# RohanVKashyap/resolution-pde

Measured on AMD Instinct MI355X. Metric: training samples/sec, FFNO2D NS 256^2, higher is better.
Workload: dtype f32; 1 GPU; FFNO2D(1,1,width=64,n_layers=4,n_modes=20,factor=4,ff_weight_norm,n_ff_layers=3,layer_norm,dropout=0.1) train step on [B,1,256,256] Gaussian random fields (BASELINE configs[2]); batch_per_gpu=32, global_batch=32, optimizer=AdamW lr=1e-3 (rpde.optim.FlatAdamW: torch.optim.AdamW's rule, one kernel), parallelism=single, grad_bucket_bytes=6828576, target=input advanced by a fixed spectral filter (utils/synthetic.py:advance)

## Files before the change

resolution-pde_amd/csrc/feedforward.hip:

```cpp
#include "rpde_internal.h"
#include "pointwise.h"
#include "gemm_kernel.h"
#include "ff_fused.h"
#include "ff_bwd_split.h"
#include "wgrad_h2.h"
#include "thin_linear.h"
#include "conv_small.h"

#include <vector>

namespace rpde {


static inline int ff_in(const rpde_ff_params* p, int l) { return l == 0 ? p->dim : p->dim * p->factor; }
static inline int ff_out(const rpde_ff_params* p, int l) { return l == p->n_layers - 1 ? p->dim : p->dim * p->factor; }

static inline int wgrad_split(long P, int out_f, int in_f) {
  const int tiles = ((out_f + 127) / 128) * ((in_f + 127) / 128);
  long s = 768 / tiles;
  const long cap = (P + 127) / 128;
  if (s > cap) s = cap;
  if (s < 1) s = 1;
  if (s > 1024) s = 1024;
  return (int)s;
// ... 86 lines not shown
  const size_t b = wgrad_h2_slab_floats(P, out_f, in_f);
  if (b > a) a = b;
  if (in_f <= 4 && thin_linear_ok(in_f, out_f) && thin_outer_ws_floats(P, in_f, out_f) > a) a = thin_outer_ws_floats(P, in_f, out_f);
  if (out_f <= 4 && thin_linear_ok(out_f, in_f) && thin_outer_ws_floats(P, out_f, in_f) > a) a = thin_outer_ws_floats(P, out_f, in_f);
  return a;
}

static rpde_ff_params ff_dims(int dim, int factor, int n_layers) {
  rpde_ff_params q;
  memset(&q, 0, sizeof(q));
  q.dim = dim; q.factor = factor; q.n_layers = n_layers;
  return q;
}
static int ff_hid(const rpde_ff_params& q) { return q.n_layers > 1 ? q.dim * q.factor : q.dim; }

struct FfBwdWork {
  float *buf0, *buf1, *small, *tailws, *dz3 = nullptr, *part = nullptr;
  void* fimg = nullptr;
  std::vector<float*> slabs, csum, wt;
  FfBwdWork(Arena& ar, const rpde_ff_params& q, long P, bool fused) {
    const int L = q.n_layers > 0 ? q.n_layers : 0, hid = ff_hid(q);
    slabs.resize(L); csum.resize(L); wt.resize(L);
    buf0 = ar.take((size_t)P * hid);
    buf1 = ar.take((size_t)P * hid);
    for (int l = 0; l < L; ++l) slabs[l] = ar.take(wgrad_ws_floats(P, ff_in(&q, l), ff_out(&q, l)));
    for (int l = 0; l < L; ++l) csum[l] = ar.take((size_t)(colsum_tiles(P) + REDUCE_CHUNKS) * hid);
    for (int l = 0; l < L; ++l) wt[l] = ar.take(ff_wimg_floats(hid));
    small = ar.take(colsum_ws_floats(P, hid));
    tailws = ar.take(ff_tail_bwd_ws_floats(P, q.dim));
    if (!fused) return;
    dz3 = ar.take((size_t)P * q.dim);
    part = ar.take(ff3_fused_bwd_part_floats());
    fimg = ar.take(ff3_fused_ws_floats());
  }
};
struct FfFwdImgs {
  std::vector<float*> wimg;
  FfFwdImgs(Arena& ar, const rpde_ff_params& q, int n) : wimg(n > 0 ? n : 0) { for (float*& w : wimg) w = ar.take(ff_wimg_floats(ff_hid(q))); }
};
struct FfFusedImg {
  void* img;
  explicit FfFusedImg(Arena& ar) : img(ar.take(ff3_fused_ws_floats())) {}
};

}

using namespace rpde;

extern "C" {

size_t rpde_feedforward_ws_bytes(int64_t P, int dim, int factor, int n_layers) {
  const rpde_ff_params q = ff_dims(dim, factor, n_layers);
  const size_t general = ws_measure<FfBwdWork>(q, (long)P, false);
  return ff3_fused_ok(&q, (long)P) ? ws_max(general, ws_measure<FfBwdWork>(q, (long)P, true)) : general;
}

size_t rpde_feedforward_fwd_ws_bytes(int dim, int factor, int n_layers) {
  return ws_max(ws_measure<FfFwdImgs>(ff_dims(dim, factor, n_layers), n_layers), ws_measure<FfFusedImg>());
}

int rpde_feedforward_is_fused(int dim, int factor, int n_layers, int64_t P) {
  const rpde_ff_params q = ff_dims(dim, factor, n_layers);
  return ff3_fused_ok(&q, (long)P) ? 1 : 0;
}

int rpde_feedforward_prepare(const rpde_ff_params* p, void* prep, size_t prep_bytes, void* stream) {
  RPDE_CHECK_ARG(p && prep, "feedforward_prepare: bad arguments");
  Arena ar(prep, prep_bytes);
  const FfFusedImg f(ar);
  RPDE_CHECK_ARG(ff3_fused_ok(p, 32) && ar.ok(), "feedforward_prepare: shape not fused or buffer too small");
  RPDE_CHECK_ARG(p->weights && p->weights[0] && p->weights[1] && p->weights[2], "feedforward_prepare: null weights");
  return ff3_fused_prepare(p, f.img, as_stream(stream));
}

int rpde_feedforward_fwd_prepared(const rpde_ff_params* p, const float* x, const float* residual, float* out, int64_t P,
                                  const void* prep, size_t prep_bytes, void* stream) {
  RPDE_CHECK_ARG(p && x && out && prep && P > 0 && P < (1L << 31), "feedforward_fwd_prepared: bad arguments");
  Arena ar(const_cast<void*>(prep), prep_bytes);
  const FfFusedImg f(ar);
  RPDE_CHECK_ARG(ff3_fused_ok(p, P) && ar.ok(), "feedforward_fwd_prepared: shape not fused");
  RPDE_CHECK_ARG(!p->layer_norm || (p->ln_gamma && p->ln_beta), "feedforward_fwd_prepared: layer_norm needs gamma/beta");
  RPDE_CHECK_ARG(p->dropout_p == 0.f, "feedforward_fwd_prepared: evaluation only");
  return ff3_fused_fwd(p, x, residual, nullptr, nullptr, out , out, P,
                       f.img, as_stream(stream), true);
}

int rpde_feedforward_fwd(const rpde_ff_params* p, const float* x, const float* residual, float* const* hs,
                         float* const* ds, float* z_last, float* out, int64_t P, void* ws, size_t ws_bytes, void* stream) {
  RPDE_CHECK_ARG(p && x && z_last && out && P > 0, "feedforward_fwd: bad arguments");
  RPDE_CHECK_ARG(p->n_layers >= 1 && p->dim > 0 && p->factor > 0, "feedforward_fwd: bad shape");
  RPDE_CHECK_ARG(P < (1L << 31), "feedforward_fwd: too many points for one call");
  RPDE_CHECK_ARG(p->dropout_p >= 0.f && p->dropout_p < 1.f, "feedforward_fwd: dropout %f", p->dropout_p);
  hipStream_t st = as_stream(stream);
  Arena far(ws, ws_bytes);
  const FfFusedImg fused(far);
  if (ff3_fused_ok(p, P) && far.ok()) {
    RPDE_CHECK_ARG(p->weights[0] && p->weights[1] && p->weights[2], "feedforward_fwd: null weights");
    RPDE_CHECK_ARG(!p->layer_norm || (p->ln_gamma && p->ln_beta), "feedforward_fwd: layer_norm needs gamma/beta");
    return ff3_fused_fwd(p, x, residual, hs, ds, z_last, out, P, fused.img, st);
  }
  RPDE_CHECK_ARG(p->n_layers == 1 || hs, "feedforward_fwd: hidden buffers missing");
  const int L = p->n_layers;
  Arena ar(ws, ws_bytes);
  bool all_imgs = ws != nullptr && L <= SplitJobs::MAX;
  const FfFwdImgs imgs(ar, *p, all_imgs ? L : 1);
  all_imgs = all_imgs && ar.ok();
  float* const* wimg = imgs.wimg.data();
  if (all_imgs) {
    SplitJobs sj;
    for (int l = 0; l < L; ++l) {
      RPDE_CHECK_ARG(p->weights[l], "feedforward_fwd: null layer %d weight", l);
      if (worth_presplit(P, ff_out(p, l), ff_in(p, l))) sj.add(p->weights[l], 1, ff_in(p, l), ff_out(p, l), ff_in(p, l), wimg[l]);
    }
    RPDE_TRY(split_weights_multi(sj, st));
  }
  for (int l = 0; l < L; ++l) {
    const bool last = l == L - 1;
    RPDE_CHECK_ARG(p->weights[l] && (last || hs[l]), "feedforward_fwd: null layer %d buffers", l);
    const float* in = l == 0 ? x : hs[l - 1];
    RPDE_TRY(linear_fwd_impl(in, p->weights[l], p->biases ? p->biases[l] : nullptr, last ? z_last : hs[l], P, ff_in(p, l),
                             ff_out(p, l), last ? RPDE_ACT_IDENTITY : RPDE_ACT_GELU, (last || !ds) ? nullptr : ds[l],
                             p->dropout_p, layer_seed(p->seed, l), st, all_imgs ? wimg[l] : wimg[0], p->seed_epoch, all_imgs));
  }
  return ff_tail_fwd(z_last, residual, out, P, p->dim, p->layer_norm, p->ln_eps, p->ln_gamma, p->ln_beta,
                     make_drop(p->dropout_p, layer_seed(p->seed, L - 1), p->seed_epoch), p->post_act, st);
}

int rpde_feedforward_bwd(const rpde_ff_params* p, const float* x, const float* const* hs, const float* const* ds,
                         const float* z_last, const float* grad_out, float* grad_x, float* const* grad_weights,
                         float* const* grad_biases, float* grad_gamma, float* grad_beta, int64_t P, void* ws,
                         size_t ws_bytes, void* stream) {
  RPDE_CHECK_ARG(p && x && z_last && grad_out && P > 0, "feedforward_bwd: bad arguments");
  RPDE_CHECK_ARG(P < (1L << 31), "feedforward_bwd: too many points for one call");
  const int L = p->n_layers;
  const int hid = ff_hid(*p);
  const bool fused = ff3_fused_ok(p, P) && hs && hs[0] && hs[1];
  RPDE_CHECK_ARG(p->n_layers == 1 || (hs && (ds || fused)), "feedforward_bwd: saved hidden tensors missing");
  RPDE_CARVE("feedforward_bwd", FfBwdWork, wk, ws, ws_bytes, *p, P, fused);
  hipStream_t st = as_stream(stream);
  float *buf0 = wk.buf0, *buf1 = wk.buf1, *small = wk.small, *tailws = wk.tailws;
  const std::vector<float*>&slabs_l = wk.slabs, &csum_l = wk.csum, &wt_l = wk.wt;
  void* wt = wt_l[0];

  if (fused) {
    const int recompute = !(ds && ds[0] && ds[1]);
    const int act_h = recompute ? RPDE_ACT_GELU : RPDE_ACT_IDENTITY;
    float *dz3 = wk.dz3, *part = wk.part;
    void* fimg = wk.fimg;
    int grid = 0;
    const bool both = grad_x && grad_weights && wgrad_h2_dgrad_ok(P, hid, p->dim);
    const bool split = both && !recompute && ff_bwd_split_ok(P, hid, p->dim);
    if (split) {
      FoldJobs folds;
      RPDE_TRY(ff_bwd_split_launch(p, ds, z_last, grad_out, x, dz3, buf0, buf1, grad_x, slabs_l[0], grad_weights[0], part,
                                   &grid, P, fimg, st, &folds));
      RPDE_TRY(linear_wgrad_impl(hs[1], dz3, grad_weights[2], nullptr, P, hid, p->dim, slabs_l[2], small, st, act_h, &folds));
      RPDE_TRY(linear_wgrad_impl(hs[0], buf0, grad_weights[1], nullptr, P, hid, hid, slabs_l[1], small, st, act_h, &folds));
      RPDE_TRY(fold_jobs(folds, st));
    } else {
      RPDE_TRY(ff3_fused_bwd_launch(p, recompute ? hs : ds, recompute, z_last, grad_out, dz3, buf0, buf1, nullptr, part, &grid, P,
                                    fimg, st));
    }
    if (grad_x && !both) RPDE_TRY(linear_dgrad_impl(buf1, p->weights[0], grad_x, P, p->dim, hid, nullptr, nullptr, st, wt));
    if (grad_weights && !split) {
      FoldJobs folds;
      RPDE_TRY(linear_wgrad_impl(hs[1], dz3, grad_weights[2], nullptr, P, hid, p->dim, slabs_l[2], small, st, act_h, &folds));
      RPDE_TRY(linear_wgrad_impl(hs[0], buf0, grad_weights[1], nullptr, P, hid, hid, slabs_l[1], small, st, act_h, &folds));
      if (both) RPDE_TRY(wgrad_h2_dgrad(buf1, x, p->weights[0], grad_weights[0], grad_x, P, p->dim, hid, slabs_l[0], st, &folds));
      else RPDE_TRY(linear_wgrad_impl(x, buf1, grad_weights[0], nullptr, P, p->dim, hid, slabs_l[0], small, st, RPDE_ACT_IDENTITY, &folds));
      RPDE_TRY(fold_jobs(folds, st));
    }
    {
      ReduceSegs sg;
      memset(&sg, 0, sizeof(sg));
      sg.n = FF3_PART; sg.nseg = 5;
      const int off[5] = {0, 256, 512, 576, 640}, len[5] = {hid, hid, p->dim, p->dim, p->dim};
      float* dst[5] = {grad_biases ? grad_biases[0] : nullptr, grad_biases ? grad_biases[1] : nullptr,
                       grad_biases ? grad_biases[2] : nullptr, p->layer_norm ? grad_gamma : nullptr,
                       p->layer_norm ? grad_beta : nullptr};
      for (int k = 0; k < 5; ++k) { sg.off[k] = off[k]; sg.len[k] = len[k]; sg.dst[k] = dst[k]; }
      RPDE_TRY(reduce_slabs_seg(part, grid, FF3_PART, sg, st));
    }
    return RPDE_OK;
  }

  FoldJobs folds;
  float* dz = buf0;
  float* other = buf1;
  int bias_done = 0;
  RPDE_TRY(ff_tail_bwd(z_last, grad_out, dz, P, p->dim, p->layer_norm, p->ln_eps, p->ln_gamma, p->ln_beta,
                       make_drop(p->dropout_p, layer_seed(p->seed, L - 1), p->seed_epoch), p->post_act, grad_gamma, grad_beta,
                       grad_biases ? grad_biases[L - 1] : nullptr, &bias_done, tailws, st, &folds));
  const bool all_imgs = L <= SplitJobs::MAX;
  if (all_imgs) {
    SplitJobs sj;
    for (int l = grad_x ? 0 : 1; l < L; ++l)
      if (worth_presplit(P, ff_in(p, l), ff_out(p, l))) sj.add(p->weights[l], 0, ff_in(p, l), ff_in(p, l), ff_out(p, l), wt_l[l]);
    RPDE_TRY(split_weights_multi(sj, st));
  }
  for (int l = L - 1; l >= 0; --l) {
    const int in_f = ff_in(p, l), out_f = ff_out(p, l);
    const float* in = l == 0 ? x : hs[l - 1];
    float* gb = (grad_biases && !bias_done) ? grad_biases[l] : nullptr;
    RPDE_TRY(linear_wgrad_impl(in, dz, grad_weights ? grad_weights[l] : nullptr, gb, P, in_f, out_f, slabs_l[l], small, st,
                               RPDE_ACT_IDENTITY, &folds));
    bias_done = 0;
    void* img = all_imgs ? wt_l[l] : wt;
    if (l > 0) {
      RPDE_CHECK_ARG(ds[l - 1], "feedforward_bwd: derivative of layer %d was not saved", l - 1);
      const bool fuse = grad_biases && can_fuse_colsum(dz, p->weights[l], other, ds[l - 1], P, in_f, out_f);
      RPDE_TRY(linear_dgrad_impl(dz, p->weights[l], other, P, in_f, out_f, ds[l - 1], fuse ? csum_l[l] : nullptr, st, img, all_imgs));
      if (fuse) {
        const int S = (int)colsum_tiles(P);
        if (!(S <= 4 * REDUCE_CHUNKS && folds.add(csum_l[l], grad_biases[l - 1], in_f, S, in_f)))
          RPDE_TRY(reduce_slabs_2pass(csum_l[l], grad_biases[l - 1], in_f, S, in_f, csum_l[l] + colsum_tiles(P) * in_f, st));
        bias_done = 1;
      }
      float* t = dz; dz = other; other = t;
    } else if (grad_x) {
      RPDE_TRY(linear_dgrad_impl(dz, p->weights[0], grad_x, P, in_f, out_f, nullptr, nullptr, st, img, all_imgs));
    }
  }
  return fold_jobs(folds, st);
}

struct LinearBwdWork {
  float *slabs, *small;
  LinearBwdWork(Arena& ar, long P, int in_f, int out_f)
      : slabs(ar.take(wgrad_ws_floats(P, in_f, out_f))), small(ar.take(colsum_ws_floats(P, out_f))) {}
};

size_t rpde_linear_ws_bytes(int64_t P, int in_f, int out_f) { return ws_measure<LinearBwdWork>((long)P, in_f, out_f); }

int rpde_linear_fwd(const float* x, const float* w, const float* b, float* out, int64_t P, int in_f, int out_f, void* stream) {
  RPDE_CHECK_ARG(x && w && out && P > 0 && in_f > 0 && out_f > 0 && P < (1L << 31), "linear_fwd: bad arguments");
  return linear_fwd_impl(x, w, b, out, P, in_f, out_f, RPDE_ACT_IDENTITY, nullptr, 0.f, 0, as_stream(stream));
}

int rpde_linear_bwd(const float* x, const float* w, const float* grad_out, float* grad_x, float* grad_w, float* grad_b,
                    int64_t P, int in_f, int out_f, void* ws, size_t ws_bytes, void* stream) {
  RPDE_CHECK_ARG(x && w && grad_out && P > 0 && in_f > 0 && out_f > 0 && P < (1L << 31), "linear_bwd: bad arguments");
  RPDE_CARVE("linear_bwd", LinearBwdWork, wk, ws, ws_bytes, P, in_f, out_f);
  hipStream_t st = as_stream(stream);
  RPDE_TRY(linear_wgrad_impl(x, grad_out, grad_w, grad_b, P, in_f, out_f, wk.slabs, wk.small, st));
  if (grad_x) RPDE_TRY(linear_dgrad_impl(grad_out, w, grad_x, P, in_f, out_f, nullptr, nullptr, st));
  return RPDE_OK;
}

static int conv1x1_ksplit(int B, int64_t S) {
  int ks = 1;
  while (ks < 8 && B * ks < 64 && S / (2 * ks) >= 128) ks *= 2;
  return ks;
}
struct Conv1x1BwdWork {
  float *slabs, *part;
  Conv1x1BwdWork(Arena& ar, int B, int Cin, int Cout, int64_t S)
      : slabs(ar.take((size_t)B * conv1x1_ksplit(B, S) * Cout * Cin)), part(ar.take((size_t)B * Cout * 64)) {}
};

size_t rpde_conv1x1_ws_bytes(int B, int Cin, int Cout, int64_t S) { return ws_measure<Conv1x1BwdWork>(B, Cin, Cout, S); }

int rpde_conv1x1_fwd(const float* x, const float* w, const float* b, float* out, int B, int Cin, int Cout, int64_t S,
                     int act_in, int accumulate, void* stream) {
  return rpde_conv1x1_act_fwd(x, w, b, out, B, Cin, Cout, S, act_in, accumulate, RPDE_ACT_IDENTITY, stream);
}

int rpde_conv1x1_act_fwd(const float* x, const float* w, const float* b, float* out, int B, int Cin, int Cout, int64_t S,
                         int act_in, int accumulate, int act_out, void* stream) {
  RPDE_CHECK_ARG(x && w && out && B > 0 && Cin > 0 && Cout > 0 && S > 0 && S < (1L << 31), "conv1x1_fwd: bad arguments");
  if (conv1x1_small_ok(x, out, Cin, Cout, S) && B <= 65535 && (long)B * S >= (1L << 20))
    return conv1x1_small(x, w, b, out, B, Cin, Cout, S, act_in, accumulate, act_out, as_stream(stream));
  rpde_gemm_desc d = gemm_desc();
  d.write_act = act_out;
  d.A = w; d.a_kmajor = 1; d.lda = Cin;
  d.B = x; d.b_kmajor = 0; d.ldb = S;
  d.C = out; d.ldc = S;
  d.M = Cout; d.N = (int)S; d.K = Cin;
  d.batch = B; d.sB1 = (long)Cin * S; d.sC1 = (long)Cout * S;
  d.bias = b; d.bias_mode = b ? 2 : 0;
  d.act_b = act_in; d.accumulate = accumulate;
  return launch_gemm(d, as_stream(stream));
}

namespace rpde {
__global__ __launch_bounds__(256) void k_rowsum(const float* __restrict__ g, float* __restrict__ part, long S) {
  __shared__ float red[256];
  const float* r = g + (long)blockIdx.x * S;
  float acc = 0.f;
  if ((S & 3) == 0 && (reinterpret_cast<uintptr_t>(r) & 15) == 0) {
    const float4* r4 = reinterpret_cast<const float4*>(r);
    for (long i = threadIdx.x; i < (S >> 2); i += 256) { const float4 v = r4[i]; acc += (v.x + v.y) + (v.z + v.w); }
  } else {
    for (long i = threadIdx.x; i < S; i += 256) acc += r[i];
  }
  red[threadIdx.x] = acc;
  __syncthreads();
  for (int w = 128; w >= 1; w >>= 1) {
    if (threadIdx.x < w) red[threadIdx.x] += red[threadIdx.x + w];
    __syncthreads();
  }
  if (threadIdx.x == 0) part[blockIdx.x] = red[0];
}
__global__ void k_fold_bias(const float* __restrict__ part, float* __restrict__ gb, int B, int C) {
  const int c = blockIdx.x * blockDim.x + threadIdx.x;
  if (c >= C) return;
  float acc = 0.f;
  for (int b = 0; b < B; ++b) acc += part[(long)b * C + c];
  gb[c] = acc;
}
// ... 44 lines not shown
```

resolution-pde_amd/csrc/ff_bwd_split.h:

```cpp
#pragma once
#include "rpde_internal.h"
#include "pointwise.h"

namespace rpde {

bool ff_bwd_split_ok(long P, int hid, int dim);

int ff_bwd_split_launch(const rpde_ff_params* p, const float* const* ds, const float* z_last, const float* grad_out,
                        const float* x, float* dz3, float* du2, float* dzb, float* gx, float* slabs, float* gw1, float* part,
                        int* grid_out, long P, void* fimg, hipStream_t st, FoldJobs* folds);

}
```

resolution-pde_amd/csrc/ff_bwd_split.hip:

```cpp
#include "ff_bwd_split.h"
#include "ff_fused.h"
#include "h2.h"
#include "pointwise.h"
#include "wgrad_h2.h"

namespace rpde {

constexpr int FS_WAVES = 8;
constexpr int FS_MAX_GRID = 256;
struct FsA {
  const float* g; const float* z3; const float* d2;
  float* dz3; float* du2; float* dzb;
  const char* wimg; const float* consts;
  const float* gamma; const float* beta;
  float* part;
  long P; int layer_norm; float eps; int post_act;
  DropCfg drop2;
  int ntiles;
};

constexpr int FA_DZBUF = 0;
constexpr int FA_VEC = FA_DZBUF + 16384;
constexpr int FA_ACC = FA_VEC + 512;
constexpr int FA_INFO = FA_ACC + 7168;
constexpr int FA_LDS = FA_INFO + 256;

__global__ __launch_bounds__(64 * FS_WAVES, 2) void k_ffs_adjoint(const FsA A0) {
  __shared__ __attribute__((aligned(16))) char smem[FA_LDS];
  FsA A = A0;
  A.drop2 = drop_resolve(A0.drop2);
  const int tid = threadIdx.x, l = tid & 63, w = tid >> 6, g = l >> 4, li = l & 15;
  f16x8 w3h[2][2], w3l[2][2];
  {
    const char* base = A.wimg + (long)w * FF3_WAVE_IMG + l * 16;
#pragma unroll
    for (int f = 0; f < 4; ++f) {
      w3h[f >> 1][f & 1] = *reinterpret_cast<const f16x8*>(base + f * 2048);
      w3l[f >> 1][f & 1] = *reinterpret_cast<const f16x8*>(base + f * 2048 + 1024);
    }
    float* vecw = reinterpret_cast<float*>(smem + FA_VEC);
    float* accw = reinterpret_cast<float*>(smem + FA_ACC);
    for (int i = tid; i < 128; i += 64 * FS_WAVES) vecw[i] = i < 64 ? (A.gamma ? A.gamma[i] : 1.f) : (A.beta ? A.beta[i - 64] : 0.f);
    for (int i = tid; i < 1792; i += 64 * FS_WAVES) accw[i] = 0.f;
  }
  const float* const vec = reinterpret_cast<const float*>(smem + FA_VEC);
  float* const acc_db2 = reinterpret_cast<float*>(smem + FA_ACC);
  float* const acc_db3 = acc_db2 + 256;
  float* const acc_dg = acc_db2 + 768;
  float* const acc_dbt = acc_db2 + 1280;
  float* const info = reinterpret_cast<float*>(smem + FA_INFO);
  const float winv3 = A.consts[2];
  const int q3 = l >> 4, feat = 4 * li;

  float4 g4n = make_float4(0.f, 0.f, 0.f, 0.f), z4n = g4n, d2n[4];
  auto issue = [&](int tile) {
    const long p = min((long)tile * 32 + 4 * w + q3, A.P - 1);
    g4n = *reinterpret_cast<const float4*>(A.g + p * 64 + feat);
    z4n = *reinterpret_cast<const float4*>(A.z3 + p * 64 + feat);
#pragma unroll
    for (int blk = 0; blk < 2; ++blk)
#pragma unroll
      for (int t = 0; t < 2; ++t)
        d2n[blk * 2 + t] = *reinterpret_cast<const float4*>(A.d2 + min((long)tile * 32 + 16 * blk + li, A.P - 1) * 256 + 16 * (2 * w + t) + 4 * g);
  };
#pragma unroll
  for (int i = 0; i < 4; ++i) d2n[i] = make_float4(0.f, 0.f, 0.f, 0.f);
  if ((int)blockIdx.x < A.ntiles) issue(blockIdx.x);
  lds_barrier();

  int par = 0;
  for (int tile = blockIdx.x; tile < A.ntiles; tile += gridDim.x, par ^= 1) {
    const int next_tile = tile + gridDim.x;
    const long p0 = (long)tile * 32;
    const int ptl = 4 * w + q3;
    const long pt3 = p0 + ptl;
    const bool live3 = pt3 < A.P;
    const long off3 = min(pt3, A.P - 1) * 64 + feat;
    const float4 g4 = g4n, z4 = z4n;
    float4 dq[4];
#pragma unroll
    for (int i = 0; i < 4; ++i) dq[i] = d2n[i];
    if (next_tile < A.ntiles) issue(next_tile);

    float s4[4] = {1.f, 1.f, 1.f, 1.f};
    if (A.drop2.on()) drop_scale4(A.drop2, (uint64_t)(pt3 * 64 + feat), s4);
    const float tz[4] = {z4.x * s4[0], z4.y * s4[1], z4.z * s4[2], z4.w * s4[3]};
    float gy[4] = {g4.x, g4.y, g4.z, g4.w};
    if (!live3) { gy[0] = gy[1] = gy[2] = gy[3] = 0.f; }
    float dz[4], dzb;
    float dgm[4] = {0.f, 0.f, 0.f, 0.f}, dbt[4] = {0.f, 0.f, 0.f, 0.f};
    if (A.layer_norm) {
      const float mean = row_all16<false>((tz[0] + tz[1]) + (tz[2] + tz[3])) * (1.f / 64.f);
      const float m2 = row_all16<false>((tz[0] - mean) * (tz[0] - mean) + (tz[1] - mean) * (tz[1] - mean) +
                                        (tz[2] - mean) * (tz[2] - mean) + (tz[3] - mean) * (tz[3] - mean));
      const float rstd = rsqrtf(m2 * (1.f / 64.f) + A.eps);
      const float4 gm = *reinterpret_cast<const float4*>(vec + feat);
      const float4 bt = *reinterpret_cast<const float4*>(vec + 64 + feat);
      const float gmv[4] = {gm.x, gm.y, gm.z, gm.w}, btv[4] = {bt.x, bt.y, bt.z, bt.w};
      float xh[4], dxh[4], s1 = 0.f, s2 = 0.f, am = 0.f;
#pragma unroll
      for (int k = 0; k < 4; ++k) {
        xh[k] = (tz[k] - mean) * rstd;
        float dy = gy[k];
        if (A.post_act) dy *= dact_f(A.post_act, xh[k] * gmv[k] + btv[k]);
        dgm[k] = dy * xh[k];
        dbt[k] = dy;
        dxh[k] = dy * gmv[k];
        s1 += dxh[k];
        s2 += dxh[k] * xh[k];
        am = fmaxf(am, fabsf(dxh[k]));
      }
      const float S1 = row_all16<false>(s1) * (1.f / 64.f), S2 = row_all16<false>(s2) * (1.f / 64.f);
      const float AM = row_all16<true>(am);
#pragma unroll
      for (int k = 0; k < 4; ++k) dz[k] = rstd * (dxh[k] - S1 - xh[k] * S2) * s4[k];
      dzb = rstd * (AM + fabsf(S1) + 8.f * fabsf(S2)) * A.drop2.scale;
    } else {
      float am = 0.f;
#pragma unroll
      for (int k = 0; k < 4; ++k) { dz[k] = gy[k] * dact_f(A.post_act, tz[k]) * s4[k]; am = fmaxf(am, fabsf(dz[k])); }
      dzb = row_all16<true>(am);
    }
    if (live3) *reinterpret_cast<float4*>(A.dz3 + off3) = make_float4(dz[0], dz[1], dz[2], dz[3]);
    {
      float b[4];
#pragma unroll
      for (int k = 0; k < 4; ++k) {
        b[k] = live3 ? dz[k] : 0.f;
        b[k] += lane_xor16(b[k]); b[k] += lane_xor32(b[k]);
        if (A.layer_norm) {
          dgm[k] += lane_xor16(dgm[k]); dgm[k] += lane_xor32(dgm[k]);
          dbt[k] += lane_xor16(dbt[k]); dbt[k] += lane_xor32(dbt[k]);
        }
      }
      if (q3 == 0) {
        float4* a3 = reinterpret_cast<float4*>(acc_db3 + w * 64 + feat);
        float4 v3 = *a3;
        v3.x += b[0]; v3.y += b[1]; v3.z += b[2]; v3.w += b[3];
        *a3 = v3;
        if (A.layer_norm) {
          float4* ag = reinterpret_cast<float4*>(acc_dg + w * 64 + feat);
          float4* ab = reinterpret_cast<float4*>(acc_dbt + w * 64 + feat);
          float4 vg = *ag, vb = *ab;
          vg.x += dgm[0]; vg.y += dgm[1]; vg.z += dgm[2]; vg.w += dgm[3];
          vb.x += dbt[0]; vb.y += dbt[1]; vb.z += dbt[2]; vb.w += dbt[3];
          *ag = vg;
          *ab = vb;
        }
      }
    }
    {
      float sdz, sdzi;
      h2_scale(dzb, 0, sdz, sdzi);
      uint2 hi, lo;
      h2_split4(dz[0] * sdz, dz[1] * sdz, dz[2] * sdz, dz[3] * sdz, hi, lo);
      const int ksz = li >> 3, cz = li & 3;
      char* dst = smem + FA_DZBUF + par * 8192 + (((ptl >> 4) * 2 + ksz) * 2) * 1024 + (cz * 16 + ((ptl & 15) ^ cz ^ (4 * ksz))) * 16 +
                  ((li >> 2) & 1) * 8;
      *reinterpret_cast<uint2*>(dst) = hi;
      *reinterpret_cast<uint2*>(dst + 1024) = lo;
      if (li == 0) {
        info[par * 32 + ptl] = dzb;
        if (live3) A.dzb[pt3] = dzb;
      }
    }
    lds_barrier();

    float bsum[8] = {0.f, 0.f, 0.f, 0.f, 0.f, 0.f, 0.f, 0.f};
#pragma unroll
    for (int blk = 0; blk < 2; ++blk) {
      const int zu = (l & 48) | ((l & 15) ^ (l >> 4));
      const char* zb = smem + FA_DZBUF + par * 8192 + (blk * 2) * 2048;
      const f16x8 zh0 = *reinterpret_cast<const f16x8*>(zb + zu * 16), zl0 = *reinterpret_cast<const f16x8*>(zb + 1024 + zu * 16);
      const f16x8 zh1 = *reinterpret_cast<const f16x8*>(zb + 2048 + (zu ^ 4) * 16), zl1 = *reinterpret_cast<const f16x8*>(zb + 3072 + (zu ^ 4) * 16);
      const long pt = p0 + 16 * blk + li;
      float sz, inv_a;
      h2_scale(info[par * 32 + blk * 16 + li], 0, sz, inv_a);
      inv_a *= winv3;
#pragma unroll
      for (int t = 0; t < 2; ++t) {
        f32x4v acc = {0.f, 0.f, 0.f, 0.f};
        acc = h2_mfma32(w3h[t][0], w3l[t][0], zh0, zl0, acc);
        acc = h2_mfma32(w3h[t][1], w3l[t][1], zh1, zl1, acc);
        const int hid = 16 * (2 * w + t) + 4 * g;
        const float4 d = dq[blk * 2 + t];
        float u[4] = {acc[0] * inv_a * d.x, acc[1] * inv_a * d.y, acc[2] * inv_a * d.z, acc[3] * inv_a * d.w};
#pragma unroll
        for (int r = 0; r < 4; ++r) pin(u[r]);
        if (pt < A.P) {
          *reinterpret_cast<float4*>(A.du2 + pt * 256 + hid) = make_float4(u[0], u[1], u[2], u[3]);
#pragma unroll
          for (int r = 0; r < 4; ++r) bsum[4 * t + r] += u[r];
        }
      }
    }
#pragma unroll
    for (int i = 0; i < 8; ++i) bsum[i] = row_sum15(bsum[i]);
    if (li == 15) {
#pragma unroll
      for (int i = 0; i < 8; ++i) acc_db2[16 * (2 * w + (i >> 2)) + 4 * g + (i & 3)] += bsum[i];
    }
  }
  lds_barrier();
  {
    float* part = A.part + (long)blockIdx.x * FF3_PART;
    for (int i = 256 + tid; i < FF3_PART; i += 64 * FS_WAVES) {
      float v;
      if (i < 512) v = acc_db2[i - 256];
      else {
        const float* a8 = acc_db3 + ((i - 512) >> 6) * 512 + ((i - 512) & 63);
        v = 0.f;
#pragma unroll
        for (int ww = 0; ww < FS_WAVES; ++ww) v += a8[ww * 64];
      }
      part[i] = v;
    }
  }
}

struct FsB {
  const float* du2; const float* d1; const float* x; const float* dzb; const float* w1;
  float* gx; float* slabs; float* part;
  const char* wimg; const float* consts;
  long P; float dmax; int ntiles;
};

constexpr int FL_PANEL = 8192;
constexpr int FL_DUBUF = 0;
constexpr int FL_PAN = FL_DUBUF + 32768;
constexpr int FL_X = FL_PAN + 4 * FL_PANEL;
constexpr int FL_W1 = FL_X + FL_PANEL;
constexpr int FL_LDS = FL_W1 + 65536;

__global__ __launch_bounds__(64 * FS_WAVES, 2) void k_ffs_layer1(const FsB A) {
  __shared__ __attribute__((aligned(16))) char smem[FL_LDS];
  __shared__ int einfo[FS_WAVES];
  __shared__ float xmax[FS_WAVES];
  __shared__ float wmax[FS_WAVES];
  __shared__ float acc_db1[256];
  const int tid = threadIdx.x, l = tid & 63, w = tid >> 6, g = l >> 4, li = l & 15;
  f16x8 w2h[2][8], w2l[2][8];
  {
    const char* base = A.wimg + (long)w * FF3_WAVE_IMG + l * 16;
#pragma unroll
    for (int f = 0; f < 16; ++f) {
      w2h[f >> 3][f & 7] = *reinterpret_cast<const f16x8*>(base + (4 + f) * 2048);
      w2l[f >> 3][f & 7] = *reinterpret_cast<const f16x8*>(base + (4 + f) * 2048 + 1024);
    }
  }
  if (tid < 256) acc_db1[tid] = 0.f;
  char* const wfrag = smem + FL_W1;
  float w_inv = 1.f;
  {
    constexpr int NF = 8 * 4 * 64 / (64 * FS_WAVES);
    float wv[NF][8];
    float m = 0.f;
#pragma unroll
    for (int r = 0; r < NF; ++r) {
      const int c = tid + r * 64 * FS_WAVES, fl = c & 63, nt = (c >> 6) & 3, ks = c >> 8;
#pragma unroll
      for (int j = 0; j < 8; ++j) {
        wv[r][j] = A.w1[(long)(32 * ks + 8 * (fl >> 4) + j) * 64 + 16 * nt + (fl & 15)];
        m = fmaxf(m, fabsf(wv[r][j]));
      }
    }
    m = wave_max(m);
    if (l == 0) wmax[w] = m;
    __syncthreads();
    m = 0.f;
#pragma unroll
    for (int i = 0; i < FS_WAVES; ++i) m = fmaxf(m, wmax[i]);
    float w_scale;
    h2_scale(m, 0, w_scale, w_inv);
#pragma unroll
    for (int r = 0; r < NF; ++r) {
      const int c = tid + r * 64 * FS_WAVES, fl = c & 63, nt = (c >> 6) & 3, ks = c >> 8;
      uint2 h0, l0, h1, l1;
      h2_split4(wv[r][0] * w_scale, wv[r][1] * w_scale, wv[r][2] * w_scale, wv[r][3] * w_scale, h0, l0);
      h2_split4(wv[r][4] * w_scale, wv[r][5] * w_scale, wv[r][6] * w_scale, wv[r][7] * w_scale, h1, l1);
      char* d = wfrag + (ks * 4 + nt) * 2048 + fl * 16;
      *reinterpret_cast<uint4*>(d) = make_uint4(h0.x, h0.y, h1.x, h1.y);
      *reinterpret_cast<uint4*>(d + 1024) = make_uint4(l0.x, l0.y, l1.x, l1.y);
    }
  }
  const float winv2 = A.consts[1], c3t = A.consts[3];

  const int xrow = tid >> 4, xc = tid & 15;
  float4 du2r[4], d1r[4], xr;
  float bzr[2];
  const unsigned cb = 32 * w + 4 * g;
  auto load_du2 = [&](int tile) {
    const long t0 = (long)tile * 32;
    const int rmax = (int)min(31L, A.P - 1 - t0);
    const float* __restrict__ src = A.du2 + t0 * 256;
    const float* __restrict__ bz = A.dzb + t0;
#pragma unroll
    for (int blk = 0; blk < 2; ++blk) {
      const unsigned r = (unsigned)min(16 * blk + li, rmax);
      bzr[blk] = bz[r];
#pragma unroll
      for (int t = 0; t < 2; ++t) du2r[blk * 2 + t] = *reinterpret_cast<const float4*>(src + (r * 256u + cb + 16u * t));
    }
  };
  auto load_d1 = [&](int tile) {
    const long t0 = (long)tile * 32;
    const int rmax = (int)min(31L, A.P - 1 - t0);
    const float* __restrict__ src = A.d1 + t0 * 256;
#pragma unroll
    for (int blk = 0; blk < 2; ++blk) {
      const unsigned r = (unsigned)min(16 * blk + li, rmax);
#pragma unroll
      for (int t = 0; t < 2; ++t) d1r[blk * 2 + t] = *reinterpret_cast<const float4*>(src + (r * 256u + cb + 16u * t));
    }
  };
  auto load_x = [&](int tile) {
    const long t0 = (long)tile * 32;
    const float* __restrict__ src = A.x + t0 * 64;
    xr = t0 + xrow < A.P ? *reinterpret_cast<const float4*>(src + (unsigned)(xrow * 64 + 4 * xc)) : make_float4(0.f, 0.f, 0.f, 0.f);
  };

  const int wm = w >> 1, wn = w & 1;
  typedef s16x4v __attribute__((address_space(3))) * lds_tr;
  f32x4v gw[4][2];
#pragma unroll
  for (int i = 0; i < 4; ++i)
#pragma unroll
    for (int j = 0; j < 2; ++j) gw[i][j] = (f32x4v){0.f, 0.f, 0.f, 0.f};
  int ea_used[2] = {15, 15}, eb_used = 15;
  int e_run = 15, e_x = 15;
  const int dg_mt = w & 1, dg_nt = w >> 1;

  if ((int)blockIdx.x < A.ntiles) { load_du2(blockIdx.x); load_d1(blockIdx.x); load_x(blockIdx.x); }
  lds_barrier();

  for (int tile = blockIdx.x; tile < A.ntiles; tile += gridDim.x) {
    const int next_tile = tile + gridDim.x;
    const bool has_next = next_tile < A.ntiles;
    const long p0 = (long)tile * 32;
    float inv_b[2];
#pragma unroll
    for (int blk = 0; blk < 2; ++blk) {
      float s_du2, ai;
      h2_scale(c3t * bzr[blk] * A.dmax, 0, s_du2, ai);
      inv_b[blk] = ai * winv2;
      const float4 a = du2r[blk * 2], b = du2r[blk * 2 + 1];
      const float hv[8] = {a.x * s_du2, a.y * s_du2, a.z * s_du2, a.w * s_du2, b.x * s_du2, b.y * s_du2, b.z * s_du2, b.w * s_du2};
      h2_put_frag(smem + FL_DUBUF + ((blk * 8 + w) * 2) * 1024 + l * 16, hv);
    }
    {
      float m = fmaxf(fmaxf(fabsf(xr.x), fabsf(xr.y)), fmaxf(fabsf(xr.z), fabsf(xr.w)));
      m = wave_max(m);
      if (l == 0) xmax[w] = m;
    }
    lds_barrier();

    float u[4][4];
    float bsum[8] = {0.f, 0.f, 0.f, 0.f, 0.f, 0.f, 0.f, 0.f};
    {
      f32x4v acc[2][2];
#pragma unroll
      for (int blk = 0; blk < 2; ++blk) {
        acc[blk][0] = (f32x4v){0.f, 0.f, 0.f, 0.f}; acc[blk][1] = (f32x4v){0.f, 0.f, 0.f, 0.f};
#pragma unroll
        for (int kap = 0; kap < 8; ++kap) {
          const char* hb = smem + FL_DUBUF + ((blk * 8 + kap) * 2) * 1024 + l * 16;
          const f16x8 bh = *reinterpret_cast<const f16x8*>(hb), bl = *reinterpret_cast<const f16x8*>(hb + 1024);
          acc[blk][0] = h2_mfma32(w2h[0][kap], w2l[0][kap], bh, bl, acc[blk][0]);
          acc[blk][1] = h2_mfma32(w2h[1][kap], w2l[1][kap], bh, bl, acc[blk][1]);
        }
      }
#pragma unroll
      for (int blk = 0; blk < 2; ++blk) {
        const bool live = p0 + 16 * blk + li < A.P;
#pragma unroll
        for (int t = 0; t < 2; ++t) {
          const float4 d4 = d1r[blk * 2 + t];
          const float d[4] = {d4.x, d4.y, d4.z, d4.w};
          float* v = u[blk * 2 + t];
          float s[4];
#pragma unroll
          for (int r = 0; r < 4; ++r) { s[r] = acc[blk][t][r] * inv_b[blk]; v[r] = s[r] * d[r]; }
          if (live) {
#pragma unroll
            for (int r = 0; r < 4; ++r) bsum[4 * t + r] = __builtin_fmaf(s[r], d[r], bsum[4 * t + r]);
          } else {
            v[0] = v[1] = v[2] = v[3] = 0.f;
          }
        }
      }
    }
    if (has_next) { load_du2(next_tile); load_d1(next_tile); }
#pragma unroll
    for (int i = 0; i < 8; ++i) bsum[i] = row_sum15(bsum[i]);
    if (li == 15) {
#pragma unroll
      for (int i = 0; i < 8; ++i) acc_db1[16 * (2 * w + (i >> 2)) + 4 * g + (i & 3)] += bsum[i];
    }
    {
      float m = 0.f;
#pragma unroll
      for (int i = 0; i < 4; ++i) m = fmaxf(fmaxf(m, fmaxf(fabsf(u[i][0]), fabsf(u[i][1]))), fmaxf(fabsf(u[i][2]), fabsf(u[i][3])));
      m = wave_max(m);
      e_run = max(e_run, (int)(__float_as_uint(m) >> 23) & 0xff);
      e_run = min(e_run, 254);
      const float scale = __uint_as_float((unsigned)(268 - e_run) << 23);
      char* const dst = smem + FL_PAN + (w >> 1) * FL_PANEL;
#pragma unroll
      for (int blk = 0; blk < 2; ++blk)
#pragma unroll
        for (int t = 0; t < 2; ++t) {
          const float* v = u[blk * 2 + t];
          uint2 hi, lo;
          h2_split4(v[0] * scale, v[1] * scale, v[2] * scale, v[3] * scale, hi, lo);
          const int off = stage_off(16 * blk + li, (w & 1) * 8 + 4 * t + g);
          *reinterpret_cast<uint2*>(dst + off) = hi;
          *reinterpret_cast<uint2*>(dst + 4096 + off) = lo;
        }
      if (l == 0) einfo[w] = e_run;
    }
    {
      float m = 0.f;
#pragma unroll
      for (int i = 0; i < FS_WAVES; ++i) m = fmaxf(m, xmax[i]);
      e_x = max(e_x, (int)(__float_as_uint(m) >> 23) & 0xff);
      e_x = min(e_x, 254);
      const float scale = __uint_as_float((unsigned)(268 - e_x) << 23);
      uint2 hi, lo;
      h2_split4(xr.x * scale, xr.y * scale, xr.z * scale, xr.w * scale, hi, lo);
      const int off = stage_off(xrow, xc);
      *reinterpret_cast<uint2*>(smem + FL_X + off) = hi;
      *reinterpret_cast<uint2*>(smem + FL_X + 4096 + off) = lo;
    }
    if (has_next) load_x(next_tile);
    lds_barrier();

    int lc = l;
    asm volatile("" : "+v"(lc));
    const int gc = lc >> 4, lic = lc & 15;
    {
      const int q = lic >> 2, pp = lic & 3;
      const int tsw = ((q >> 1) & 1) | ((gc & 1) << 1);
      const int trow = (8 * gc + q) * 128 + pp * 8;
      auto frag = [&](const char* panel, int tile, f16x8& hi, f16x8& lo) {
        const char* t = panel + trow + ((tile ^ tsw) << 5);
        union { struct { s16x4v a, b; } h; f16x8 v; } uh, ul;
        uh.h.a = __builtin_amdgcn_ds_read_tr16_b64_v4i16((lds_tr)(t));
        uh.h.b = __builtin_amdgcn_ds_read_tr16_b64_v4i16((lds_tr)(t + 512));
        ul.h.a = __builtin_amdgcn_ds_read_tr16_b64_v4i16((lds_tr)(t + 4096));
        ul.h.b = __builtin_amdgcn_ds_read_tr16_b64_v4i16((lds_tr)(t + 4096 + 512));
        hi = uh.v; lo = ul.v;
      };
      const int eb = __builtin_amdgcn_readfirstlane(e_x);
#pragma unroll
      for (int k = 0; k < 2; ++k) {
        const int ea = __builtin_amdgcn_readfirstlane(einfo[2 * wm + k]);
        if (ea + eb != ea_used[k] + eb_used) {
          const int d = (ea_used[k] + eb_used) - (ea + eb);
          const float f = d > -126 ? __uint_as_float((unsigned)(127 + d) << 23) : 0.f;
#pragma unroll
          for (int j = 0; j < 2; ++j) { gw[2 * k][j] *= f; gw[2 * k + 1][j] *= f; }
        }
        ea_used[k] = ea;
      }
      eb_used = eb;
      f16x8 bh[2], bl[2];
#pragma unroll
      for (int j = 0; j < 2; ++j) frag(smem + FL_X, 2 * wn + j, bh[j], bl[j]);
#pragma unroll
      for (int i = 0; i < 4; ++i) {
        f16x8 ah, al;
        frag(smem + FL_PAN + wm * FL_PANEL, i, ah, al);
#pragma unroll
        for (int j = 0; j < 2; ++j) gw[i][j] = h2_mfma32(ah, al, bh[j], bl[j], gw[i][j]);
      }
    }
    {
      f32x4v tot = (f32x4v){0.f, 0.f, 0.f, 0.f};
      const int row = 16 * dg_mt + lic;
#pragma unroll
      for (int hp = 0; hp < 8; ++hp) {
        const char* pa_ = smem + FL_PAN + (hp >> 1) * FL_PANEL + stage_off(row, 2 * (4 * (hp & 1) + gc));
        const f16x8 ah = *reinterpret_cast<const f16x8*>(pa_), al = *reinterpret_cast<const f16x8*>(pa_ + 4096);
        const char* wb = wfrag + (hp * 4 + dg_nt) * 2048 + lc * 16;
        const f16x8 bh = *reinterpret_cast<const f16x8*>(wb), bl = *reinterpret_cast<const f16x8*>(wb + 1024);
        const f32x4v part = h2_mfma32(ah, al, bh, bl, (f32x4v){0.f, 0.f, 0.f, 0.f});
        const int ek = __builtin_amdgcn_readfirstlane(einfo[hp]);
        const float fk = __uint_as_float((unsigned)(ek - 14) << 23) * w_inv;
        tot += part * fk;
      }
      float t0 = tot[0], t1 = tot[1], t2 = tot[2], t3 = tot[3];
      quad_transpose(t0, t1, t2, t3);
      const int rq = 16 * dg_mt + 4 * gc + (lic & 3);
      if (p0 + rq < A.P) *reinterpret_cast<float4*>(A.gx + p0 * 64 + (unsigned)(rq * 64 + 16 * dg_nt + 4 * (lic >> 2))) = make_float4(t0, t1, t2, t3);
    }
  }

  const float fb = __uint_as_float((unsigned)(eb_used - 14) << 23);
  float* __restrict__ out = A.slabs + (long)blockIdx.x * 256 * 64;
  const unsigned o0 = (unsigned)((wm * 64 + 4 * g) * 64 + wn * 32 + li);
#pragma unroll
  for (int i = 0; i < 4; ++i) {
    const float fa = __uint_as_float((unsigned)(ea_used[i >> 1] - 14) << 23);
#pragma unroll
    for (int j = 0; j < 2; ++j)
#pragma unroll
      for (int r = 0; r < 4; ++r) out[o0 + (unsigned)((16 * i + r) * 64 + 16 * j)] = gw[i][j][r] * fa * fb;
  }
  lds_barrier();
  if (tid < 256) A.part[(long)blockIdx.x * FF3_PART + tid] = acc_db1[tid];
}

bool ff_bwd_split_ok(long P, int hid, int dim) { return !switch_off("RPDE_FF_BWD_SPLIT") && wgrad_h2_dgrad_ok(P, hid, dim); }

int ff_bwd_split_launch(const rpde_ff_params* p, const float* const* ds, const float* z_last, const float* grad_out,
                        const float* x, float* dz3, float* du2, float* dzb, float* gx, float* slabs, float* gw1, float* part,
                        int* grid_out, long P, void* fimg, hipStream_t st, FoldJobs* folds) {
  RPDE_CHECK_ARG(ff_bwd_split_ok(P, p->dim * p->factor, p->dim) && ds && ds[0] && ds[1] && gx && gw1 && slabs,
                 "ff_bwd_split: unsupported call");
  const char* img;
  const float* consts;
  RPDE_TRY(ff3_fused_bwd_prepare(p, fimg, &img, &consts, st));
  const int ntiles = (int)((P + 31) / 32);
  int cus;
  RPDE_HIP(cu_count(&cus));
  int grid = cus < FS_MAX_GRID ? cus : FS_MAX_GRID;
  if (ntiles < grid) grid = ntiles;
  const DropCfg drop2 = make_drop(p->dropout_p, layer_seed(p->seed, 2), p->seed_epoch);

  FsA a;
  memset(&a, 0, sizeof(a));
  a.g = grad_out; a.z3 = z_last; a.d2 = ds[1];
  a.dz3 = dz3; a.du2 = du2; a.dzb = dzb;
  a.wimg = img; a.consts = consts; a.gamma = p->ln_gamma; a.beta = p->ln_beta; a.part = part;
  a.P = P; a.layer_norm = p->layer_norm; a.eps = p->ln_eps; a.post_act = p->post_act;
  a.drop2 = drop2; a.ntiles = ntiles;
  hipLaunchKernelGGL(k_ffs_adjoint, dim3(grid), dim3(64 * FS_WAVES), 0, st, a);
  RPDE_LAUNCH_CHECK();

  FsB b;
  memset(&b, 0, sizeof(b));
  b.du2 = du2; b.d1 = ds[0]; b.x = x; b.dzb = dzb; b.w1 = p->weights[0];
  b.gx = gx; b.slabs = slabs; b.part = part;
  b.wimg = img; b.consts = consts;
  b.P = P; b.dmax = 1.13f * drop2.scale;
  b.ntiles = ntiles;
  hipLaunchKernelGGL(k_ffs_layer1, dim3(grid), dim3(64 * FS_WAVES), 0, st, b);
  RPDE_LAUNCH_CHECK();
  *grid_out = grid;
  const int hid = p->dim * p->factor;
  if (folds && folds->add(slabs, gw1, hid * p->dim, grid, (long)hid * p->dim)) return RPDE_OK;
  return reduce_slabs(slabs, gw1, (long)hid * p->dim, grid, (long)hid * p->dim, 1.f, 0, st);
}

}
```

Measured before the change: 1065 samples/s.

## Fuse layer-3 weight gradient into FFN backward adjoint kernel

The adjoint kernel now computes the last FF layer's weight gradient (dz3 x h2) in place. It stages dz3 and h2 tiles into LDS as split-f16 panels and accumulates with MFMA across tiles, writing per-block slabs. This removes the global dz3 write and the separate linear_wgrad_impl launch that reread dz3 and h2. In exchange it adds LDS use (an extra 48KB per block), registers and extra h2 loads inside the adjoint kernel, which could lower occupancy.

```diff
diff --git a/resolution-pde_amd/csrc/feedforward.hip b/resolution-pde_amd/csrc/feedforward.hip
--- a/resolution-pde_amd/csrc/feedforward.hip
+++ b/resolution-pde_amd/csrc/feedforward.hip
@@ -262,9 +262,8 @@
     const bool split = both && !recompute && ff_bwd_split_ok(P, hid, p->dim);
     if (split) {
       FoldJobs folds;
-      RPDE_TRY(ff_bwd_split_launch(p, ds, z_last, grad_out, x, dz3, buf0, buf1, grad_x, slabs_l[0], grad_weights[0], part,
-                                   &grid, P, fimg, st, &folds));
-      RPDE_TRY(linear_wgrad_impl(hs[1], dz3, grad_weights[2], nullptr, P, hid, p->dim, slabs_l[2], small, st, act_h, &folds));
+      RPDE_TRY(ff_bwd_split_launch(p, ds, hs[1], z_last, grad_out, x, buf0, buf1, grad_x, slabs_l[0], grad_weights[0],
+                                   slabs_l[2], grad_weights[2], part, &grid, P, fimg, st, &folds));
       RPDE_TRY(linear_wgrad_impl(hs[0], buf0, grad_weights[1], nullptr, P, hid, hid, slabs_l[1], small, st, act_h, &folds));
       RPDE_TRY(fold_jobs(folds, st));
     } else {
diff --git a/resolution-pde_amd/csrc/ff_bwd_split.h b/resolution-pde_amd/csrc/ff_bwd_split.h
--- a/resolution-pde_amd/csrc/ff_bwd_split.h
+++ b/resolution-pde_amd/csrc/ff_bwd_split.h
@@ -6,8 +6,9 @@
 
 bool ff_bwd_split_ok(long P, int hid, int dim);
 
-int ff_bwd_split_launch(const rpde_ff_params* p, const float* const* ds, const float* z_last, const float* grad_out,
-                        const float* x, float* dz3, float* du2, float* dzb, float* gx, float* slabs, float* gw1, float* part,
-                        int* grid_out, long P, void* fimg, hipStream_t st, FoldJobs* folds);
+int ff_bwd_split_launch(const rpde_ff_params* p, const float* const* ds, const float* h2, const float* z_last,
+                        const float* grad_out, const float* x, float* du2, float* dzb, float* gx, float* slabs, float* gw1,
+                        float* slabs3, float* gw3, float* part, int* grid_out, long P, void* fimg, hipStream_t st,
+                        FoldJobs* folds);
 
 }
diff --git a/resolution-pde_amd/csrc/ff_bwd_split.hip b/resolution-pde_amd/csrc/ff_bwd_split.hip
--- a/resolution-pde_amd/csrc/ff_bwd_split.hip
+++ b/resolution-pde_amd/csrc/ff_bwd_split.hip
@@ -7,10 +7,11 @@
 namespace rpde {
 
 constexpr int FS_WAVES = 8;
+constexpr int FS_PANEL = 8192;
 constexpr int FS_MAX_GRID = 256;
 struct FsA {
-  const float* g; const float* z3; const float* d2;
-  float* dz3; float* du2; float* dzb;
+  const float* g; const float* z3; const float* d2; const float* h2;
+  float* du2; float* dzb; float* slabs;
   const char* wimg; const float* consts;
   const float* gamma; const float* beta;
   float* part;
@@ -23,7 +24,10 @@
 constexpr int FA_VEC = FA_DZBUF + 16384;
 constexpr int FA_ACC = FA_VEC + 512;
 constexpr int FA_INFO = FA_ACC + 7168;
-constexpr int FA_LDS = FA_INFO + 256;
+constexpr int FA_DZMAX = FA_INFO + 256;
+constexpr int FA_DZPAN = FA_DZMAX + 256;
+constexpr int FA_HPAN = FA_DZPAN + 2 * FS_PANEL;
+constexpr int FA_LDS = FA_HPAN + 4 * FS_PANEL;
 
 __global__ __launch_bounds__(64 * FS_WAVES, 2) void k_ffs_adjoint(const FsA A0) {
   __shared__ __attribute__((aligned(16))) char smem[FA_LDS];
@@ -49,10 +53,11 @@
   float* const acc_dg = acc_db2 + 768;
   float* const acc_dbt = acc_db2 + 1280;
   float* const info = reinterpret_cast<float*>(smem + FA_INFO);
+  float* const dzmax = reinterpret_cast<float*>(smem + FA_DZMAX);
   const float winv3 = A.consts[2];
   const int q3 = l >> 4, feat = 4 * li;
 
-  float4 g4n = make_float4(0.f, 0.f, 0.f, 0.f), z4n = g4n, d2n[4];
+  float4 g4n = make_float4(0.f, 0.f, 0.f, 0.f), z4n = g4n, d2n[4], h2n[4];
   auto issue = [&](int tile) {
     const long p = min((long)tile * 32 + 4 * w + q3, A.P - 1);
     g4n = *reinterpret_cast<const float4*>(A.g + p * 64 + feat);
@@ -63,10 +68,91 @@
       for (int t = 0; t < 2; ++t)
         d2n[blk * 2 + t] = *reinterpret_cast<const float4*>(A.d2 + min((long)tile * 32 + 16 * blk + li, A.P - 1) * 256 + 16 * (2 * w + t) + 4 * g);
   };
-#pragma unroll
-  for (int i = 0; i < 4; ++i) d2n[i] = make_float4(0.f, 0.f, 0.f, 0.f);
-  if ((int)blockIdx.x < A.ntiles) issue(blockIdx.x);
+  auto issue_h2 = [&](int tile) {
+#pragma unroll
+    for (int blk = 0; blk < 2; ++blk)
+#pragma unroll
+      for (int t = 0; t < 2; ++t)
+        h2n[blk * 2 + t] = *reinterpret_cast<const float4*>(A.h2 + min((long)tile * 32 + 16 * blk + li, A.P - 1) * 256 + 16 * (2 * w + t) + 4 * g);
+  };
+#pragma unroll
+  for (int i = 0; i < 4; ++i) d2n[i] = h2n[i] = make_float4(0.f, 0.f, 0.f, 0.f);
+  if ((int)blockIdx.x < A.ntiles) { issue(blockIdx.x); issue_h2(blockIdx.x); }
   lds_barrier();
+
+  f32x4v gw[4][2];
+#pragma unroll
+  for (int i = 0; i < 4; ++i)
+#pragma unroll
+    for (int j = 0; j < 2; ++j) gw[i][j] = (f32x4v){0.f, 0.f, 0.f, 0.f};
+  int e_h = 15, e_dz = 15;
+  int ea_used = 15, eb_used = 15;
+  typedef s16x4v __attribute__((address_space(3))) * lds_tr;
+  auto gw3_products = [&](int pp, int ea, int eb) {
+    if (ea + eb != ea_used + eb_used) {
+      const int d = (ea_used + eb_used) - (ea + eb);
+      const float f = d > -126 ? __uint_as_float((unsigned)(127 + d) << 23) : 0.f;
+#pragma unroll
+      for (int i = 0; i < 4; ++i)
+#pragma unroll
+        for (int j = 0; j < 2; ++j) gw[i][j] *= f;
+    }
+    ea_used = ea; eb_used = eb;
+    int lc = l;
+    asm volatile("" : "+v"(lc));
+    const int gc = lc >> 4, lic = lc & 15;
+    const int q = lic >> 2, pq = lic & 3;
+    const int tsw = ((q >> 1) & 1) | ((gc & 1) << 1);
+    const int trow = (8 * gc + q) * 128 + pq * 8;
+    auto frag = [&](const char* panel, int tile, f16x8& hi, f16x8& lo) {
+      const char* t = panel + trow + ((tile ^ tsw) << 5);
+      union { struct { s16x4v a, b; } h; f16x8 v; } uh, ul;
+      uh.h.a = __builtin_amdgcn_ds_read_tr16_b64_v4i16((lds_tr)(t));
+      uh.h.b = __builtin_amdgcn_ds_read_tr16_b64_v4i16((lds_tr)(t + 512));
+      ul.h.a = __builtin_amdgcn_ds_read_tr16_b64_v4i16((lds_tr)(t + 4096));
+      ul.h.b = __builtin_amdgcn_ds_read_tr16_b64_v4i16((lds_tr)(t + 4096 + 512));
+      hi = uh.v; lo = ul.v;
+    };
+    const char* const hpan = smem + FA_HPAN + (w >> 1) * FS_PANEL;
+    const char* const zpan = smem + FA_DZPAN + pp * FS_PANEL;
+    f16x8 bh[2], bl[2];
+#pragma unroll
+    for (int j = 0; j < 2; ++j) frag(hpan, 2 * (w & 1) + j, bh[j], bl[j]);
+#pragma unroll
+    for (int i = 0; i < 4; ++i) {
+      f16x8 ah, al;
+      frag(zpan, i, ah, al);
+#pragma unroll
+      for (int j = 0; j < 2; ++j) gw[i][j] = h2_mfma32(ah, al, bh[j], bl[j], gw[i][j]);
+    }
+    asm volatile("" ::: "memory");
+  };
+  auto stage_h2 = [&](long p0) {
+    if (p0 + 32 > A.P) {
+#pragma unroll
+      for (int blk = 0; blk < 2; ++blk)
+        if (p0 + 16 * blk + li >= A.P) h2n[blk * 2] = h2n[blk * 2 + 1] = make_float4(0.f, 0.f, 0.f, 0.f);
+    }
+    float m = 0.f;
+#pragma unroll
+    for (int i = 0; i < 4; ++i) m = fmaxf(fmaxf(m, fmaxf(fabsf(h2n[i].x), fabsf(h2n[i].y))), fmaxf(fabsf(h2n[i].z), fabsf(h2n[i].w)));
+    m = wave_max(m);
+    e_h = max(e_h, (int)(__float_as_uint(m) >> 23) & 0xff);
+    e_h = min(e_h, 254);
+    const float scale = __uint_as_float((unsigned)(268 - e_h) << 23);
+    char* const dst = smem + FA_HPAN + (w >> 1) * FS_PANEL;
+#pragma unroll
+    for (int blk = 0; blk < 2; ++blk)
+#pragma unroll
+      for (int t = 0; t < 2; ++t) {
+        const float4 h = h2n[blk * 2 + t];
+        uint2 hi, lo;
+        h2_split4(h.x * scale, h.y * scale, h.z * scale, h.w * scale, hi, lo);
+        const int off = stage_off(16 * blk + li, (w & 1) * 8 + 4 * t + g);
+        *reinterpret_cast<uint2*>(dst + off) = hi;
+        *reinterpret_cast<uint2*>(dst + 4096 + off) = lo;
+      }
+  };
 
   int par = 0;
   for (int tile = blockIdx.x; tile < A.ntiles; tile += gridDim.x, par ^= 1) {
@@ -75,7 +161,6 @@
     const int ptl = 4 * w + q3;
     const long pt3 = p0 + ptl;
     const bool live3 = pt3 < A.P;
-    const long off3 = min(pt3, A.P - 1) * 64 + feat;
     const float4 g4 = g4n, z4 = z4n;
     float4 dq[4];
 #pragma unroll
@@ -121,7 +206,6 @@
       for (int k = 0; k < 4; ++k) { dz[k] = gy[k] * dact_f(A.post_act, tz[k]) * s4[k]; am = fmaxf(am, fabsf(dz[k])); }
       dzb = row_all16<true>(am);
     }
-    if (live3) *reinterpret_cast<float4*>(A.dz3 + off3) = make_float4(dz[0], dz[1], dz[2], dz[3]);
     {
       float b[4];
 #pragma unroll
@@ -164,7 +248,29 @@
         if (live3) A.dzb[pt3] = dzb;
       }
     }
+    float dzp[4];
+    {
+#pragma unroll
+      for (int k = 0; k < 4; ++k) dzp[k] = live3 ? dz[k] : 0.f;
+      const float m = wave_max(fmaxf(fmaxf(fabsf(dzp[0]), fabsf(dzp[1])), fmaxf(fabsf(dzp[2]), fabsf(dzp[3]))));
+      if (l == 0) dzmax[par * FS_WAVES + w] = m;
+    }
     lds_barrier();
+
+    const int e_dz_prev = e_dz;
+    {
+      float m = 0.f;
+#pragma unroll
+      for (int i = 0; i < FS_WAVES; ++i) m = fmaxf(m, dzmax[par * FS_WAVES + i]);
+      e_dz = max(e_dz, (int)(__float_as_uint(m) >> 23) & 0xff);
+      e_dz = __builtin_amdgcn_readfirstlane(min(e_dz, 254));
+      const float scale = __uint_as_float((unsigned)(268 - e_dz) << 23);
+      uint2 hi, lo;
+      h2_split4(dzp[0] * scale, dzp[1] * scale, dzp[2] * scale, dzp[3] * scale, hi, lo);
+      const int off = stage_off(ptl, li);
+      *reinterpret_cast<uint2*>(smem + FA_DZPAN + par * FS_PANEL + off) = hi;
+      *reinterpret_cast<uint2*>(smem + FA_DZPAN + par * FS_PANEL + 4096 + off) = lo;
+    }
 
     float bsum[8] = {0.f, 0.f, 0.f, 0.f, 0.f, 0.f, 0.f, 0.f};
 #pragma unroll
@@ -200,8 +306,23 @@
 #pragma unroll
       for (int i = 0; i < 8; ++i) acc_db2[16 * (2 * w + (i >> 2)) + 4 * g + (i & 3)] += bsum[i];
     }
+    if (tile != (int)blockIdx.x) gw3_products(par ^ 1, e_dz_prev, e_h);
+    stage_h2(p0);
+    if (next_tile < A.ntiles) issue_h2(next_tile);
   }
   lds_barrier();
+  if ((int)blockIdx.x < A.ntiles) gw3_products(par ^ 1, e_dz, e_h);
+  {
+    const float fa = __uint_as_float((unsigned)(ea_used - 14) << 23), fb = __uint_as_float((unsigned)(eb_used - 14) << 23);
+    float* __restrict__ out = A.slabs + (long)blockIdx.x * 64 * 256;
+    const unsigned o0 = (unsigned)(4 * g * 256 + 32 * w + li);
+#pragma unroll
+    for (int i = 0; i < 4; ++i)
+#pragma unroll
+      for (int j = 0; j < 2; ++j)
+#pragma unroll
+        for (int r = 0; r < 4; ++r) out[o0 + (unsigned)((16 * i + r) * 256 + 16 * j)] = gw[i][j][r] * fa * fb;
+  }
   {
     float* part = A.part + (long)blockIdx.x * FF3_PART;
     for (int i = 256 + tid; i < FF3_PART; i += 64 * FS_WAVES) {
@@ -225,11 +346,10 @@
   long P; float dmax; int ntiles;
 };
 
-constexpr int FL_PANEL = 8192;
 constexpr int FL_DUBUF = 0;
 constexpr int FL_PAN = FL_DUBUF + 32768;
-constexpr int FL_X = FL_PAN + 4 * FL_PANEL;
-constexpr int FL_W1 = FL_X + FL_PANEL;
+constexpr int FL_X = FL_PAN + 4 * FS_PANEL;
+constexpr int FL_W1 = FL_X + FS_PANEL;
 constexpr int FL_LDS = FL_W1 + 65536;
 
 __global__ __launch_bounds__(64 * FS_WAVES, 2) void k_ffs_layer1(const FsB A) {
@@ -404,7 +524,7 @@
       e_run = max(e_run, (int)(__float_as_uint(m) >> 23) & 0xff);
       e_run = min(e_run, 254);
       const float scale = __uint_as_float((unsigned)(268 - e_run) << 23);
-      char* const dst = smem + FL_PAN + (w >> 1) * FL_PANEL;
+      char* const dst = smem + FL_PAN + (w >> 1) * FS_PANEL;
 #pragma unroll
       for (int blk = 0; blk < 2; ++blk)
 #pragma unroll
@@ -469,7 +589,7 @@
 #pragma unroll
       for (int i = 0; i < 4; ++i) {
         f16x8 ah, al;
-        frag(smem + FL_PAN + wm * FL_PANEL, i, ah, al);
+        frag(smem + FL_PAN + wm * FS_PANEL, i, ah, al);
 #pragma unroll
         for (int j = 0; j < 2; ++j) gw[i][j] = h2_mfma32(ah, al, bh[j], bl[j], gw[i][j]);
       }
@@ -479,7 +599,7 @@
       const int row = 16 * dg_mt + lic;
 #pragma unroll
       for (int hp = 0; hp < 8; ++hp) {
-        const char* pa_ = smem + FL_PAN + (hp >> 1) * FL_PANEL + stage_off(row, 2 * (4 * (hp & 1) + gc));
+        const char* pa_ = smem + FL_PAN + (hp >> 1) * FS_PANEL + stage_off(row, 2 * (4 * (hp & 1) + gc));
         const f16x8 ah = *reinterpret_cast<const f16x8*>(pa_), al = *reinterpret_cast<const f16x8*>(pa_ + 4096);
         const char* wb = wfrag + (hp * 4 + dg_nt) * 2048 + lc * 16;
         const f16x8 bh = *reinterpret_cast<const f16x8*>(wb), bl = *reinterpret_cast<const f16x8*>(wb + 1024);
@@ -512,10 +632,11 @@
 
 bool ff_bwd_split_ok(long P, int hid, int dim) { return !switch_off("RPDE_FF_BWD_SPLIT") && wgrad_h2_dgrad_ok(P, hid, dim); }
 
-int ff_bwd_split_launch(const rpde_ff_params* p, const float* const* ds, const float* z_last, const float* grad_out,
-                        const float* x, float* dz3, float* du2, float* dzb, float* gx, float* slabs, float* gw1, float* part,
-                        int* grid_out, long P, void* fimg, hipStream_t st, FoldJobs* folds) {
-  RPDE_CHECK_ARG(ff_bwd_split_ok(P, p->dim * p->factor, p->dim) && ds && ds[0] && ds[1] && gx && gw1 && slabs,
+int ff_bwd_split_launch(const rpde_ff_params* p, const float* const* ds, const float* h2, const float* z_last,
+                        const float* grad_out, const float* x, float* du2, float* dzb, float* gx, float* slabs, float* gw1,
+                        float* slabs3, float* gw3, float* part, int* grid_out, long P, void* fimg, hipStream_t st,
+                        FoldJobs* folds) {
+  RPDE_CHECK_ARG(ff_bwd_split_ok(P, p->dim * p->factor, p->dim) && ds && ds[0] && ds[1] && h2 && gx && gw1 && slabs && gw3 && slabs3,
                  "ff_bwd_split: unsupported call");
   const char* img;
   const float* consts;
@@ -529,8 +650,8 @@
 
   FsA a;
   memset(&a, 0, sizeof(a));
-  a.g = grad_out; a.z3 = z_last; a.d2 = ds[1];
-  a.dz3 = dz3; a.du2 = du2; a.dzb = dzb;
+  a.g = grad_out; a.z3 = z_last; a.d2 = ds[1]; a.h2 = h2;
+  a.du2 = du2; a.dzb = dzb; a.slabs = slabs3;
   a.wimg = img; a.consts = consts; a.gamma = p->ln_gamma; a.beta = p->ln_beta; a.part = part;
   a.P = P; a.layer_norm = p->layer_norm; a.eps = p->ln_eps; a.post_act = p->post_act;
   a.drop2 = drop2; a.ntiles = ntiles;
@@ -548,8 +669,10 @@
   RPDE_LAUNCH_CHECK();
   *grid_out = grid;
   const int hid = p->dim * p->factor;
-  if (folds && folds->add(slabs, gw1, hid * p->dim, grid, (long)hid * p->dim)) return RPDE_OK;
-  return reduce_slabs(slabs, gw1, (long)hid * p->dim, grid, (long)hid * p->dim, 1.f, 0, st);
+  const long n = (long)hid * p->dim;
+  if (!(folds && folds->add(slabs, gw1, (int)n, grid, n))) RPDE_TRY(reduce_slabs(slabs, gw1, n, grid, n, 1.f, 0, st));
+  if (folds && folds->add(slabs3, gw3, (int)n, grid, n)) return RPDE_OK;
+  return reduce_slabs(slabs3, gw3, n, grid, n, 1.f, 0, st);
 }
 
 }
```

New measurement: 1075 samples/s (median of 6 runs). About the same (+1.0%).
